# quzefan/LuSh-NeRF

Measured on AMD Instinct MI355X. Metric: training rays/sec (fwd+bwd), N_samples=64+64, higher is better.
Workload: dtype f16 MFMA forward (one fp16 plane per operand, fp32 accumulate; render outputs within 3e-5 of the fp32 reference); backward fp16 MFMA (one plane, per-launch power-of-two loss scale), fp32 accumulate; 1 GPU; poster_lushnerf 1xMI355X N_rand=4096/GPU N_samples=64 N_importance=64 blur kernel (DSK/RBK) on, fwd+bwd+Adam, one RCCL all-reduce of the flat gradient (BASELINE config C2); rays_per_gpu=4096, marched_rays_per_gpu=20480, planes_fwd=fp16x1, parallelism=dp1

## Files before the change

lush_nerf_amd/csrc/lush_abi.hip:

```cpp
#include "lush_common.h"
#include "lush_host.h"
#include <cstring>
#include <vector>
#include "../../include/lush_march.h"

using namespace lush;

namespace {

struct NetInfo { int HW, NL, SKIP, HV, NRB, total_entries, f32_total; };
template <class N> NetInfo info_of() { return {N::HW, N::NL, N::SKIP, N::HV, N::NRB, N::total_entries, N::f32_total}; }
bool net_info(int net, NetInfo& o) {
    if (net == 0) { o = info_of<NetNerf>(); return true; }
    if (net == 1) { o = info_of<NetNoise>(); return true; }
    return false;
}

inline bool code_ok(int c) { return (c >= 1 && c <= 3) || c == PLANES_F16; }
inline int nplanes(int c) { return c == PLANES_F16 ? 1 : c; }
constexpr int PT_PAD = 256;
inline long long pad_pts(long long P) { return (P + PT_PAD - 1) / PT_PAD * PT_PAD; }
inline size_t al256(size_t x) { return (x + 255) & ~(size_t)255; }

struct StashLayout {
    size_t mask, mask_dummy, pe, xd, h[NET_MAX_LAYERS], feat, hv, total;
    long long Ppad;
};
StashLayout stash_layout(const NetInfo& n, int pf, int sp, long long P) {
    StashLayout L{};
    L.Ppad = pad_pts(P);
    size_t off = 0;
    L.mask = off; off += sp ? al256((size_t)(L.Ppad / 32) * (n.NL + 1) * n.NRB * 16 * 8) : 0;
    L.mask_dummy = off; off += sp ? 4096 : 0;
    for (int l = 0; l < n.NL; ++l) { L.h[l] = off; off += al256((size_t)sp * L.Ppad * n.HW * 2); }
    L.feat = off; off += sp >= 3 ? al256((size_t)sp * L.Ppad * n.HW * 2) : 0;
    L.hv = off;   off += al256((size_t)sp * L.Ppad * n.HV * 2);
    L.xd = off;   off += sp ? al256((size_t)L.Ppad * 32) : 0;
    L.pe = off;   off += al256((size_t)pf * L.Ppad * PE_ROW * 2);
    L.total = off;
    return L;
}
struct DStashLayout { size_t scale, fac, dz[NET_MAX_LAYERS], dfeat, dzv, total; };
DStashLayout dstash_layout(const NetInfo& n, int ns, long long P) {
    DStashLayout L{};
    const long long Ppad = pad_pts(P);
    size_t off = 0;
    L.scale = off; off += 256;
    L.fac = off; off += ns <= 2 ? al256((size_t)((n.HV + DZV_EXT) * (n.HW + 1) + DZV_EXT * (n.HV + 1)) * 4) : 0;
    for (int l = 0; l < n.NL; ++l) { L.dz[l] = off; off += al256((size_t)ns * Ppad * n.HW * 2); }
    L.dfeat = off; off += ns >= 3 ? al256((size_t)ns * Ppad * n.HW * 2) : 0;
    L.dzv = off;   off += al256((size_t)ns * Ppad * (n.HV + (ns == 1 ? DZV_EXT : 0)) * 2);
    L.total = off;
    return L;
}

MlpParams to_params(const lush_mlp_params* p) {
    MlpParams q;
    for (int i = 0; i < NET_MAX_LAYERS; ++i) { q.w[i] = p->w[i]; q.b[i] = p->b[i]; }
    q.w_feat = p->w_feat; q.b_feat = p->b_feat; q.w_alpha = p->w_alpha; q.b_alpha = p->b_alpha;
    q.w_views = p->w_views; q.b_views = p->b_views; q.w_rgb = p->w_rgb; q.b_rgb = p->b_rgb;
    return q;
}

template <class N>
void build_pack_table(const lush_mlp_params* p, PackTable& T, int& blocks, int copy_lo, int copy_hi) {
    constexpr int HW = N::HW, HV = N::HV, NL = N::NL, SK = N::SKIP;
    T.n = 0;
    blocks = 0;
    int perm = 0, base = 0;
    auto add = [&](const float* src, int sr, int sk, int rows, int cols, int nrb, int kk, int dst) {
        PackJob& j = T.j[T.n++];
        j.src = src; j.sr = sr; j.sk = sk; j.rows = rows; j.cols = cols; j.nrb = nrb; j.kk = kk; j.perm = perm;
        j.dst_entry = base + dst; j.first_block = blocks;
        blocks += nrb * kk;
    };
    const int XV = PE_X_VALID, DV = PE_D_VALID;
    for (int copy = copy_lo; copy <= copy_hi; ++copy) {
        perm = copy; base = copy ? N::fwd2_base : 0;
        add(p->w[0], XV, 1, HW, XV, N::NRB, N::KKX, N::fwd_L(0, false));
        for (int l = 1; l < NL; ++l) {
            if (l == SK) {
                add(p->w[l], XV + HW, 1, HW, XV, N::NRB, N::KKX, N::fwd_L(l, false));
                add(p->w[l] + XV, XV + HW, 1, HW, HW, N::NRB, N::KKH, N::fwd_L(l, true));
            } else {
                add(p->w[l], HW, 1, HW, HW, N::NRB, N::KKH, N::fwd_L(l, true));
            }
        }
        add(p->w_feat, HW, 1, HW, HW, N::NRB, N::KKH, N::fwd_FEAT);
        add(p->w_alpha, HW, 1, 1, HW, 1, N::KKH, N::fwd_ALPHA);
        add(p->w_views, HW + DV, 1, HV, HW, N::NRBV, N::KKH, N::fwd_VA);
        add(p->w_views + HW, HW + DV, 1, HV, DV, N::NRBV, N::KKD, N::fwd_VB);
        add(p->w_rgb, HV, 1, 3, HV, 1, N::KKV, N::fwd_RGB);
    }
    perm = 0; base = 0;
    for (int copy = copy_lo; copy <= copy_hi; ++copy) {
        perm = copy; base = copy ? N::bwd2_base - N::bwd_VAT : 0;
        add(p->w_views, 1, HW + DV, HW, HV, N::NRB, N::KKV, N::bwd_VAT);
        add(p->w_views + HW, 1, HW + DV, DV, HV, 1, N::KVB, N::bwd_VBT);
        add(p->w_feat, 1, HW, HW, HW, N::NRB, N::KKH, N::bwd_FEATT);
        for (int l = NL - 1; l >= 1; --l) {
            if (l == SK) {
                add(p->w[l], 1, XV + HW, XV, HW, 2, N::KKH, N::bwd_LT(l, false));
                add(p->w[l] + XV, 1, XV + HW, HW, HW, N::NRB, N::KKH, N::bwd_LT(l, true));
            } else {
                add(p->w[l], 1, HW, HW, HW, N::NRB, N::KKH, N::bwd_LT(l, true));
            }
        }
        add(p->w[0], 1, XV, XV, HW, 2, N::KKH, N::bwd_LT(0, false));
    }
    perm = 0; base = 0;
}

template <class N>
void build_pack_table_half(const lush_mlp_params* p, PackTable& T, int& blocks) {
    constexpr int HW = N::HW, HV = N::HV, NL = N::NL, SK = N::SKIP, HR = N::HW / 2, NRBH = N::NRB / 2;
    T.n = 0;
    blocks = 0;
    int dst = N::fwd3_base;
    auto add = [&](const float* src, int sr, int rows, int cols, int nrb, int kk) {
        PackJob& j = T.j[T.n++];
        j.src = src; j.sr = sr; j.sk = 1; j.rows = rows; j.cols = cols; j.nrb = nrb; j.kk = kk; j.perm = 1;
        j.dst_entry = dst; j.first_block = blocks;
        blocks += nrb * kk;
        dst += nrb * kk;
    };
    const int XV = PE_X_VALID, DV = PE_D_VALID;
    for (int half = 0; half < 2; ++half) add(p->w[0] + (long long)half * HR * XV, XV, HR, XV, NRBH, N::KKX);
    for (int l = 1; l < NL; ++l) {
        const int ld = l == SK ? XV + HW : HW;
        for (int half = 0; half < 2; ++half) {
            const float* w = p->w[l] + (long long)half * HR * ld;
            if (l == SK) {
                add(w, ld, HR, XV, NRBH, N::KKX);
                add(w + XV, ld, HR, HW, NRBH, N::KKH);
            } else {
                add(w, ld, HR, HW, NRBH, N::KKH);
            }
        }
    }
    for (int half = 0; half < 2; ++half) add(p->w_feat + (long long)half * HR * HW, HW, HR, HW, NRBH, N::KKH);
    add(p->w_alpha, HW, 1, HW, 1, N::KKH);
    add(p->w_views, HW + DV, HV, HW, N::NRBV, N::KKH);
    add(p->w_views + HW, HW + DV, HV, DV, N::NRBV, N::KKD);
    add(p->w_rgb, HV, 3, HV, 1, N::KKV);
}

template <class N>
void build_pack_table_wide(const lush_mlp_params* p, PackTable& T, int& blocks) {
    constexpr int HW = N::HW, HV = N::HV, NL = N::NL, SK = N::SKIP, QR = 64;
    T.n = 0;
    blocks = 0;
    int dst = N::fwd4_base;
    auto add = [&](const float* src, int sr, int rows, int cols, int nrb, int kk) {
        PackJob& j = T.j[T.n++];
        j.src = src; j.sr = sr; j.sk = 1; j.rows = rows; j.cols = cols; j.nrb = nrb; j.kk = kk; j.perm = 1;
        j.dst_entry = dst; j.first_block = blocks;
        blocks += nrb * kk;
        dst += nrb * kk;
    };
    const int XV = PE_X_VALID, DV = PE_D_VALID;
    for (int q = 0; q < HW / QR; ++q) add(p->w[0] + (long long)q * QR * XV, XV, QR, XV, 2, N::KKX);
    for (int l = 1; l < NL; ++l) {
        const int ld = l == SK ? XV + HW : HW;
        for (int q = 0; q < HW / QR; ++q) {
            const float* w = p->w[l] + (long long)q * QR * ld;
            if (l == SK) {
                add(w, ld, QR, XV, 2, N::KKX);
                add(w + XV, ld, QR, HW, 2, N::KKH);
            } else {
                add(w, ld, QR, HW, 2, N::KKH);
            }
        }
    }
    for (int q = 0; q < HW / QR; ++q) add(p->w_feat + (long long)q * QR * HW, HW, QR, HW, 2, N::KKH);
    add(p->w_alpha, HW, 1, HW, 1, N::KKH);
    for (int q = 0; q < HV / QR; ++q) {
        const float* w = p->w_views + (long long)q * QR * (HW + DV);
        add(w + HW, HW + DV, QR, DV, 2, 4);
        add(w, HW + DV, QR, HW, 2, N::KKH);
    }
    add(p->w_rgb, HV, 3, HV, 1, N::KKV);
}

template <class N>
void build_pack_table_wide_bwd(const lush_mlp_params* p, PackTable& T, int& blocks) {
    constexpr int HW = N::HW, HV = N::HV, NL = N::NL, SK = N::SKIP, QR = 64;
    T.n = 0;
    blocks = 0;
    int dst = N::bwd4_base;
    auto add = [&](const float* src, int sk, int rows, int cols, int nrb, int kk) {
        PackJob& j = T.j[T.n++];
        j.src = src; j.sr = 1; j.sk = sk; j.rows = rows; j.cols = cols; j.nrb = nrb; j.kk = kk; j.perm = 1;
        j.dst_entry = dst; j.first_block = blocks;
        blocks += nrb * kk;
        dst += nrb * kk;
    };
    const int XV = PE_X_VALID, DV = PE_D_VALID;
    for (int q = 0; q < HW / QR; ++q) add(p->w_views + q * QR, HW + DV, QR, HV, 2, N::KKV);
    add(p->w_views + HW, HW + DV, DV, HV, 1, N::KKV);
    for (int q = 0; q < HW / QR; ++q) add(p->w_feat + q * QR, HW, QR, HW, 2, N::KKH);
    for (int l = NL - 1; l >= 1; --l) {
        const int ld = l == SK ? XV + HW : HW;
        for (int q = 0; q < HW / QR; ++q) add(p->w[l] + (l == SK ? XV : 0) + q * QR, ld, QR, HW, 2, N::KKH);
        if (l == SK) add(p->w[l], ld, XV, HW, 2, N::KKH);
    }
    add(p->w[0], XV, XV, HW, 2, N::KKH);
}

template <class N>
void build_pack_table_half_bwd(const lush_mlp_params* p, PackTable& T, int& blocks) {
    constexpr int HW = N::HW, HV = N::HV, NL = N::NL, SK = N::SKIP, HR = N::HW / 2, NRBH = N::NRB / 2;
    T.n = 0;
    blocks = 0;
    int dst = N::bwd3_base;
    auto add = [&](const float* src, int sk, int rows, int cols, int nrb, int kk) {
        PackJob& j = T.j[T.n++];
        j.src = src; j.sr = 1; j.sk = sk; j.rows = rows; j.cols = cols; j.nrb = nrb; j.kk = kk; j.perm = 1;
        j.dst_entry = dst; j.first_block = blocks;
        blocks += nrb * kk;
        dst += nrb * kk;
    };
    const int XV = PE_X_VALID, DV = PE_D_VALID;
    for (int half = 0; half < 2; ++half) add(p->w_views + half * HR, HW + DV, HR, HV, NRBH, N::KKV);
    add(p->w_views + HW, HW + DV, DV, HV, 1, N::KVB);
    for (int half = 0; half < 2; ++half) add(p->w_feat + half * HR, HW, HR, HW, NRBH, N::KKH);
    for (int l = NL - 1; l >= 1; --l) {
        const int ld = l == SK ? XV + HW : HW;
        if (l == SK) add(p->w[l], ld, XV, HW, 2, N::KKH);
        for (int half = 0; half < 2; ++half) add(p->w[l] + (l == SK ? XV : 0) + half * HR, ld, HR, HW, NRBH, N::KKH);
    }
    add(p->w[0], XV, XV, HW, 2, N::KKH);
}

int dw_splits(long long Ppad) {
    int dev = 0, s = 256;
    if (current_device_cus(dev, s) != 0) s = 256;
#ifndef LUSH_DW_MIN_PTS
#define LUSH_DW_MIN_PTS 128
#endif
    const long long max_s = Ppad / LUSH_DW_MIN_PTS > 0 ? Ppad / LUSH_DW_MIN_PTS : 1;
    if (s > max_s) s = (int)max_s;
    return s < 1 ? 1 : s;
}

}

extern "C" {

size_t lush_mlp_packed_bytes(int net, int planes) {
    NetInfo n;
    if (!net_info(net, n) || !code_ok(planes)) return 0;
    return al256((size_t)n.total_entries * nplanes(planes) * 1024 + (size_t)n.f32_total * 4);
}

static int collect_pack_tables(int net, int planes, const lush_mlp_params* prm, int variant, std::vector<PackTable>& out,
                               std::vector<int>& out_blocks) {
    if (!code_ok(planes)) return set_error("lush_mlp_pack: planes must be 1..3 or 17 (fp16)");
    if (net != 0 && net != 1) return set_error("lush_mlp_pack: bad net");
    auto push = [&](const PackTable& T, int blocks) { out.push_back(T); out_blocks.push_back(blocks); };
    PackTable T;
    int blocks = 0;
    const int older = LUSH_VARIANT_FWD_HALF | LUSH_VARIANT_FWD_512 | LUSH_VARIANT_BWD_HALF | LUSH_VARIANT_BWD_512;
    if (net == 0 && planes == PLANES_F16 && variant >= 0 && !(variant & older)) {
        build_pack_table_wide<NetNerf>(prm, T, blocks);
        if (blocks != NetNerf::fwd4_len) return set_error("lush_mlp_pack: quarter-row stream length");
        push(T, blocks);
        build_pack_table_wide_bwd<NetNerf>(prm, T, blocks);
        if (blocks != NetNerf::bwd4_len) return set_error("lush_mlp_pack: transposed quarter-row stream length");
        push(T, blocks);
        return 0;
    }
    const bool fc = mlp_fwd_chain_enabled(planes), bc = mlp_bwd_chain_enabled(planes);
    const int lo = (fc && bc) ? 1 : 0, hi = (fc || bc) ? 1 : 0;
    if (net == 0) build_pack_table<NetNerf>(prm, T, blocks, lo, hi);
    else build_pack_table<NetNoise>(prm, T, blocks, lo, hi);
    push(T, blocks);
    if (net == 0 && nplanes(planes) == 1) {
        build_pack_table_half<NetNerf>(prm, T, blocks);
        push(T, blocks);
        if (planes == PLANES_F16) {
            build_pack_table_half_bwd<NetNerf>(prm, T, blocks);
            push(T, blocks);
            build_pack_table_wide<NetNerf>(prm, T, blocks);
            if (blocks != NetNerf::fwd4_len) return set_error("lush_mlp_pack: quarter-row stream length");
            push(T, blocks);
            build_pack_table_wide_bwd<NetNerf>(prm, T, blocks);
            if (blocks != NetNerf::bwd4_len) return set_error("lush_mlp_pack: transposed quarter-row stream length");
            push(T, blocks);
        }
    }
    return 0;
}

int lush_mlp_pack_for(int net, int planes, const lush_mlp_params* prm, void* packed, int variant, lush_stream_t stream) {
    std::vector<PackTable> tables;
    std::vector<int> blocks;
    int rc = collect_pack_tables(net, planes, prm, variant, tables, blocks);
    for (size_t i = 0; i < tables.size() && !rc; ++i) rc = launch_pack(planes, tables[i], blocks[i], packed, (hipStream_t)stream);
    if (rc) return rc;
    return launch_pack_f32(net, nplanes(planes), to_params(prm), packed, (hipStream_t)stream);
// ... 444 lines not shown
```

lush_nerf_amd/csrc/lush_mlp.h:

```cpp
#pragma once
#include <stdint.h>

namespace lush {

enum { NET_MAX_LAYERS = 8 };
enum { PLANES_F16 = 17 };
enum { LUSH_VARIANT_FWD_HALF = 1, LUSH_VARIANT_FWD_512 = 2, LUSH_VARIANT_BWD_512 = 4, LUSH_VARIANT_HEAD_KERNEL = 8, LUSH_VARIANT_BWD_HALF = 16,
       LUSH_VARIANT_PE_ROWS = 64, LUSH_VARIANT_DW_SPLIT = 128, LUSH_VARIANT_DENSE_BWD = 256, LUSH_VARIANT_DW_WALK = 512,
       LUSH_VARIANT_KERNEL_BITS = 0x3DF };

template <int HW_, int NL_, int SKIP_>
struct NetT {
    static constexpr int HW = HW_, NL = NL_, SKIP = SKIP_;
    static constexpr int HV = HW / 2;
    static constexpr int NRB = HW / 32, NRBV = HV / 32;
    static constexpr int KKH = HW / 16, KKV = HV / 16;
    static constexpr int KKX = 4, KKD = 2;

    static constexpr int fwd_L(int l, bool part_b) {
        int off = 0;
        if (l == 0) return 0;
        off += KKX * NRB;
        for (int i = 1; i < l; ++i) off += (i == SKIP ? (KKX + KKH) : KKH) * NRB;
        if (l == SKIP && part_b) off += KKX * NRB;
        return off;
    }
    static constexpr int fwd_FEAT = fwd_L(NL, false);
    static constexpr int fwd_ALPHA = fwd_FEAT + KKH * NRB;
    static constexpr int fwd_VA = fwd_ALPHA + KKH;
    static constexpr int fwd_VB = fwd_VA + KKH * NRBV;
    static constexpr int fwd_RGB = fwd_VB + KKD * NRBV;
    static constexpr int fwd_END = fwd_RGB + KKV;

    static constexpr int KVB = 2 * NRB;
    static_assert(KVB >= KKV && KVB <= KKH, "VBT padding");
    static constexpr int bwd_VAT = fwd_END;
    static constexpr int bwd_VBT = bwd_VAT + KKV * NRB;
    static constexpr int bwd_FEATT = bwd_VBT + KVB;
    static constexpr int bwd_LT(int l, bool part_b) {
        int off = bwd_FEATT + KKH * NRB;
        for (int i = NL - 1; i > l; --i) off += (i == SKIP ? (KKH * 2 + KKH * NRB) : KKH * NRB);
        if (l == SKIP && part_b) off += KKH * 2;
        return off;
    }
    static constexpr int bwd_END = bwd_LT(0, false) + KKH * 2;
    static constexpr int fwd2_base = bwd_END;
    static constexpr int bwd2_base = fwd2_base + fwd_END;
    static constexpr int fwd3_base = bwd2_base + (bwd_END - bwd_VAT);
    static constexpr int bwd3_base = fwd3_base + fwd_END;
    static constexpr int fwd4_base = bwd3_base + (bwd_END - bwd_VAT);
    static constexpr int fwd4_len = fwd_ALPHA + KKH + (HV / 64) * (8 + 2 * KKH) + KKV;
    static constexpr int bwd4_base = fwd4_base + fwd4_len;
    static constexpr int bwd4_len = (HW / 64) * 2 * KKV + KKV + (HW / 64) * 2 * KKH * NL + (SKIP > 0 ? 2 * KKH : 0) + 2 * KKH;
    static constexpr int total_entries = bwd4_base + bwd4_len;

    static constexpr int n_mask_layers = NL + 1;

    static constexpr int f32_b_trunk = 0;
    static constexpr int f32_b_feat = NL * HW;
    static constexpr int f32_b_alpha = f32_b_feat + HW;
    static constexpr int f32_b_views = f32_b_alpha + 32;
    static constexpr int f32_b_rgb = f32_b_views + HV;
    static constexpr int f32_w_rgb = f32_b_rgb + 32;
    static constexpr int f32_w_alpha = f32_w_rgb + 3 * HV;
    static constexpr int f32_total = f32_w_alpha + HW;
};

typedef NetT<256, 8, 5> NetNerf;
typedef NetT<128, 4, -1> NetNoise;

__host__ __device__ constexpr int chain_row(int rho) {
    const int h = (rho >> 2) & 1, q = (rho & 3) + 4 * (rho >> 3);
    return 16 * (q >> 3) + 8 * h + (q & 7);
}

struct PackJob {
    const float* src;
    int sr, sk;
    int rows, cols;
    int nrb, kk;
    int perm;
    int dst_entry;
    int first_block;
};

struct PackTable {
    PackJob j[64];
    int n;
};

struct PlanJob {
    PackJob j;
    void* dst;
    int code;
    int kind;
    int prm_index;
    int pad;
};
constexpr int PLAN_MAX_NETS = 8;
struct PlanHeader {
    int n_jobs, total_blocks, n_prm, pad;
};

struct MlpParams {
    const float* w[NET_MAX_LAYERS];
    const float* b[NET_MAX_LAYERS];
    const float *w_feat, *b_feat, *w_alpha, *b_alpha, *w_views, *b_views, *w_rgb, *b_rgb;
};

struct MlpGrads {
    float* w[NET_MAX_LAYERS];
    float* b[NET_MAX_LAYERS];
    float *w_feat, *b_feat, *w_alpha, *b_alpha, *w_views, *b_views, *w_rgb, *b_rgb;
};

struct MlpFwdArgs {
    const float* rays;
    const float* z;
    int S, P, n_tiles;
    const uint4* wpk;
    float* raw;
    unsigned long long* mask;
    void* mask_dummy;
    __bf16* pe;
    float* xd;
    int pe_rows;
    __bf16* h0;
    __bf16* feat;
    __bf16* hv;
    long long h_stride;
    long long plane_pe, plane_h, plane_hv;
    int write_stash;
    int stash_planes;
    const int* live_idx;
    const int* live_cnt;
};

struct MlpBwdArgs {
    const float* rays;
    const float* z;
    int S, P, n_tiles;
    const uint4* wpk;
    const float* draw;
    const unsigned long long* mask;
    __bf16* dz0;
    __bf16* dfeat;
    __bf16* dzv;
    long long dz_stride;
    long long plane_h, plane_hv;
    float* dpts;
    const float* scale;
    const int* live_idx;
    const int* live_cnt;
};

struct DwArgs {
    const __bf16* Z; long long z_plane; int ldz; int n_out;
    const __bf16* X; long long x_plane; int ldx; int xcol0; int k_in;
    float* dW; int ldw; int wcol0;
    float* db;
    int x_f16;
    int z_f16;
    const float* scale;
    int Ppad;
    int pts_per_split;
};

// ... 48 lines not shown
```

lush_nerf_amd/csrc/lush_mlp.hip:

```cpp
#include "lush_common.h"
#include "lush_mlp.h"
#include "lush_mlp_dev.h"

namespace lush {

constexpr int DW_THREADS = 256;

template <int NS, int DT>
__device__ __forceinline__ void pack_entry(const PackJob& J, int e, __bf16* __restrict__ dst) {
    const int kk = e / J.nrb, rb = e % J.nrb;
    const int lane = threadIdx.x, r = lane & 31, h = lane >> 5;
    const int row = rb * 32 + (J.perm ? chain_row(r) : r);
    __bf16 out[NS][8];
#pragma unroll
    for (int i = 0; i < 8; ++i) {
        const int k = kk * 16 + 8 * h + i;
        float v = 0.f;
        if (row < J.rows && k < J.cols) v = J.src[(long long)row * J.sr + (long long)k * J.sk];
        __bf16 p[NS];
        split_planes<NS, DT>(v, p);
#pragma unroll
        for (int s = 0; s < NS; ++s) out[s][i] = p[s];
    }
    __bf16* base = dst + ((long long)(J.dst_entry + e) * NS) * 64 * 8;
#pragma unroll
    for (int s = 0; s < NS; ++s) {
        bf16x8 v;
#pragma unroll
        for (int i = 0; i < 8; ++i) v[i] = out[s][i];
        *reinterpret_cast<bf16x8*>(base + ((long long)s * 64 + lane) * 8) = v;
    }
}

template <int NS, int DT>
__global__ __launch_bounds__(64) void pack_kernel(const PackTable T, __bf16* __restrict__ dst) {
    int b = blockIdx.x;
    int j = 0;
    while (j + 1 < T.n && T.j[j + 1].first_block <= b) ++j;
    const PackJob J = T.j[j];
    pack_entry<NS, DT>(J, b - J.first_block, dst);
}

template <class N>
__device__ __forceinline__ float pack_f32_value(const MlpParams& P, int i) {
    float v = 0.f;
    if (i < N::f32_b_feat) v = P.b[i / N::HW][i % N::HW];
    else if (i < N::f32_b_alpha) v = P.b_feat[i - N::f32_b_feat];
    else if (i < N::f32_b_views) v = (i == N::f32_b_alpha) ? P.b_alpha[0] : 0.f;
    else if (i < N::f32_b_rgb) v = P.b_views[i - N::f32_b_views];
    else if (i < N::f32_w_rgb) v = (i - N::f32_b_rgb < 3) ? P.b_rgb[i - N::f32_b_rgb] : 0.f;
    else if (i < N::f32_w_alpha) v = P.w_rgb[i - N::f32_w_rgb];
    else v = P.w_alpha[i - N::f32_w_alpha];
    return v;
}
template <class N>
__global__ void pack_f32_kernel(const MlpParams P, float* __restrict__ dst) {
    const int i = blockIdx.x * blockDim.x + threadIdx.x;
    if (i >= N::f32_total) return;
    dst[i] = pack_f32_value<N>(P, i);
}

__global__ __launch_bounds__(64) void pack_plan_kernel(const PlanHeader* __restrict__ H, float* __restrict__ zero_buf, long long zero_n) {
    if (zero_buf != nullptr) {
        const long long t = (long long)blockIdx.x * 64 + threadIdx.x, nt = (long long)gridDim.x * 64;
        if ((reinterpret_cast<size_t>(zero_buf) & 15) == 0) {
            float4* z4 = reinterpret_cast<float4*>(zero_buf);
            for (long long i = t; i < zero_n / 4; i += nt) z4[i] = make_float4(0.f, 0.f, 0.f, 0.f);
            for (long long i = zero_n / 4 * 4 + t; i < zero_n; i += nt) zero_buf[i] = 0.f;
        } else {
            for (long long i = t; i < zero_n; i += nt) zero_buf[i] = 0.f;
        }
    }
    const MlpParams* prm = reinterpret_cast<const MlpParams*>(H + 1);
    const PlanJob* jobs = reinterpret_cast<const PlanJob*>(prm + PLAN_MAX_NETS);
    const int b = blockIdx.x;
    int lo = 0, hi = H->n_jobs - 1;
    while (lo < hi) {
        const int mid = (lo + hi + 1) >> 1;
        if (jobs[mid].j.first_block <= b) lo = mid; else hi = mid - 1;
    }
    const PlanJob& PJ = jobs[lo];
    const int e = b - PJ.j.first_block;
    if (PJ.kind == 0) {
        const PackJob J = PJ.j;
        __bf16* dst = reinterpret_cast<__bf16*>(PJ.dst);
        if (PJ.code == PLANES_F16) pack_entry<1, DT_F16>(J, e, dst);
        else if (PJ.code == 1) pack_entry<1, DT_BF16>(J, e, dst);
        else if (PJ.code == 2) pack_entry<2, DT_BF16>(J, e, dst);
        else pack_entry<3, DT_BF16>(J, e, dst);
    } else {
        const int i = e * 64 + threadIdx.x;
        float* dst = reinterpret_cast<float*>(PJ.dst);
        if (PJ.kind == 1) { if (i < NetNerf::f32_total) dst[i] = pack_f32_value<NetNerf>(prm[PJ.prm_index], i); }
        else if (i < NetNoise::f32_total) dst[i] = pack_f32_value<NetNoise>(prm[PJ.prm_index], i);
    }
}

template <int NS, int RB, int CB, int KK, int DT = DT_BF16>
__device__ __forceinline__ void seg_gemm(f32x16 (&acc)[RB][CB], const bf16x8* __restrict__ wseg,
                                         int nrb, int rb0, const char* img, int plane_bytes,
                                         int row_bytes, int chunk0, int lane) {
// ... 1617 lines not shown
```

lush_nerf_amd/csrc/lush_mlp_wide_bwd.hip:

```cpp
#include "lush_mlp_wide.h"
#include "lush_host.h"

#include <cstdio>
#include <cstdlib>

namespace lush {

constexpr int WB_WRAP = NetNerf::bwd4_len / 8;
LUSH_CLOCK_DECL(lush_clock_wide_bwd)
#ifdef LUSH_PROF
__device__ unsigned long long lush_prof_wbwd[16];
#define BPROF_T(var) const unsigned long long var = __builtin_amdgcn_s_memtime()
#define BPROF_ADD(slot, t0) cx.prof[slot] += __builtin_amdgcn_s_memtime() - (t0)
#else
#define BPROF_T(var)
#define BPROF_ADD(slot, t0)
#endif
static_assert(NetNerf::bwd4_len % 8 == 0, "the transposed quarter-row stream is whole positions");
constexpr int WB_DPE_LD = 104;
constexpr int WB_TILE_OPS = 6 + 32 + 2 + 16;
constexpr int WB_SB = 2;
enum { WK_NONE = 0, WK_ACT = 1, WK_ID = 2 };

struct WbRt {
    unsigned mrd;
    const float* initw;
    float dalpha[2];
    const char* msrc[2];
    unsigned mdst;
    char* tile;
    const char* lut;
    char* srows;
    unsigned srow_off;
};

struct WbConvTmp {
    unsigned w[4];
    u32x4 Y[2];
    unsigned o[4];
};

enum { WI_L = 0, WI_P = 1, WI_ID = 2, WI_IA = 3, WI_IB = 4 };
struct WbItem { int kind, b, t, i; };

template <int NRQ, int NPOS, int CK, int CKB0, bool INIT, bool ZERO, int D, int PQ, bool STASH, int LD, bool MDMA, int XP = 0>
struct WbPass {
    static constexpr int KBPP = 8 / NRQ;
    static constexpr int NG = NPOS * 16;
    static constexpr int DG = D < NG ? D : NG;
    struct Seq { WbItem it[128]; int n; };
    static constexpr Seq make_seq() {
        Seq q{};
        q.n = 0;
        auto put = [&](int kind, int b, int t, int i) { q.it[q.n].kind = kind; q.it[q.n].b = b; q.it[q.n].t = t; q.it[q.n].i = i; ++q.n; };
        auto init = [&](int b) {
            if (INIT) {
                for (int j = 0; j < 4; ++j) put(WI_IA, b, 0, j);
                for (int j = 0; j < 4; ++j) put(WI_IB, b, 0, j);
            }
        };
        if (CK == WK_ACT) {
            put(WI_L, 0, 0, 0);
            for (int bt = 0; bt < 8; ++bt) {
                if (bt + 1 < 8) put(WI_L, (bt + 1) / 2, (bt + 1) % 2, 0);
                for (int i = 0; i < 4; ++i) put(WI_P, bt / 2, bt % 2, i);
                if (bt % 2 == 1) init(bt / 2);
            }
        } else if (CK == WK_ID) {
            for (int bt = 0; bt < 8; ++bt) {
                for (int i = 0; i < 4; ++i) put(WI_ID, bt / 2, bt % 2, i);
                if (bt % 2 == 1) init(bt / 2);
            }
        } else {
            for (int b = 0; b < 4; ++b) init(b);
        }
        return q;
    }
    static constexpr Seq SQ = make_seq();
    static constexpr int NIT = SQ.n;
    static constexpr int START = CK == WK_ACT ? 2 : 0;
    static_assert(!STASH || NPOS == 4, "the stash pipeline is laid out over the 16 positions of a layer");

    struct Regs {
        bf16x8 a1[4];
        WbConvTmp ct;
        unsigned dma_dst, dma_off;
    };

    static constexpr int ST_JOBS = 8;
    static constexpr bool st_write(int g) { return STASH && g % 16 >= 12 && (4 * PQ + g / 16) < ST_JOBS; }
    static constexpr bool st_read(int g) { return STASH && g % 16 >= 12 && (4 * PQ + g / 16) >= 1 && (4 * PQ + g / 16) <= ST_JOBS; }
// ... 330 lines not shown
        const unsigned voff_row = (unsigned)(((lane >> 3) * LD_ + (lane & 7) * 8) * 2);
#pragma unroll
        for (int i = 0; i < 4; ++i) {
            const int row = 8 * i + (lane >> 3);
            const u32x4 v = *reinterpret_cast<const u32x4*>(rt.tile + row * 128 + (((lane & 7) ^ (row & 7)) << 4));
            asm volatile("global_store_dwordx4 %0, %1, %2 nt\n\ts_nop 1" ::"v"(voff_row), "v"(v), "s"(rows + ((c * 32 + 8 * i) * LD_ + j * 64) * 2) : "memory");
        }
    };

    f32x4 drn[2];
    auto prefetch = [&](int t) __attribute__((always_inline)) {
        const long long wp = (long long)t * WD_MT + row0;
        const char* mb0 = wd_uniform(reinterpret_cast<const char*>(A.mask) + (wp / 32) * CB_BYTES - w * 1024);
        wd_dma_pair(mb0 + NL * 1024, mb0 + CB_BYTES + NL * 1024, cx.voff, mbuf_lds + (NL % 2) * 2048u, mbuf_lds + (NL % 2) * 2048u + 1024u);
        wd_dma_pair(mb0 + (NL - 1) * 1024, mb0 + CB_BYTES + (NL - 1) * 1024, cx.voff, mbuf_lds + ((NL - 1) % 2) * 2048u, mbuf_lds + ((NL - 1) % 2) * 2048u + 1024u);
#pragma unroll
        for (int c = 0; c < 2; ++c) {
            long long gpt = wp + c * 32 + n;
            if (gpt >= P) gpt = P - 1;
            asm volatile("global_load_dwordx4 %0, %1, %2" : "=v"(drn[c]) : "v"((unsigned)(gpt * 16)), "s"(A.draw) : "memory");
        }
    };
    if ((int)blockIdx.x < n_tiles) prefetch(blockIdx.x);
    asm volatile("s_waitcnt vmcnt(0)" : "+v"(drn[0]), "+v"(drn[1])::"memory");
#ifdef LUSH_PROF
    for (int i = 0; i < 16; ++i) cx.prof[i] = 0;
    const unsigned long long t_kernel = __builtin_amdgcn_s_memtime();
#endif

    for (int tile = blockIdx.x; tile < n_tiles; tile += gridDim.x) {
        const long long pt0 = (long long)tile * WD_MT;
        const long long wpt = pt0 + row0;
        BPROF_T(t_tile);
        {
            unsigned long long gb = (unsigned long long)cx.gbase;
            asm volatile("" : "+s"(gb));
            cx.gbase = (const char*)gb;
        }
        const char* mbase[2];
#pragma unroll
        for (int c = 0; c < 2; ++c) mbase[c] = wd_uniform(reinterpret_cast<const char*>(A.mask) + (wpt / 32 + c) * CB_BYTES - w * 1024);
        asm volatile("s_waitcnt vmcnt(32)" : "+v"(drn[0]), "+v"(drn[1])::"memory");
        float4 dr[2];
#pragma unroll
        for (int c = 0; c < 2; ++c) {
            const bool in = wpt + c * 32 + n < P;
            dr[c].x = in ? drn[c][0] * gscale : 0.f; dr[c].y = in ? drn[c][1] * gscale : 0.f;
            dr[c].z = in ? drn[c][2] * gscale : 0.f; dr[c].w = in ? drn[c][3] * gscale : 0.f;
            rt.dalpha[c] = dr[c].w;
        }
        BPROF_ADD(1, t_tile);
        BPROF_T(t_bar);
        lds_barrier();
        BPROF_ADD(2, t_bar);
        BPROF_T(t_pro);

        f32x16 accA[2][2], accB[2][2];
        u32x4 B0[2][16], B1[2][16];
        WdCarry a0;
#pragma unroll
        for (int i = 0; i < 4; ++i) a0.a0[i] = *reinterpret_cast<const bf16x8*>(cx.ring + cx.slot_off + i * 1024 + cx.voff);

#ifndef LUSH_ABL_NOPRO
        {
            auto rank3 = [&](f32x16 (&acc)[2][2], int r0) __attribute__((always_inline)) {
#pragma unroll
                for (int rbl = 0; rbl < 2; ++rbl)
#pragma unroll
                    for (int j = 0; j < 4; ++j) {
                        const int f = r0 + rbl * 32 + 8 * h + (j == 0 ? 0 : j == 1 ? 4 : j == 2 ? 16 : 20);
                        const f32x4 wr = *reinterpret_cast<const f32x4*>(w_rgb + f);
                        const f32x4 wg = *reinterpret_cast<const f32x4*>(w_rgb + HV + f);
                        const f32x4 wb = *reinterpret_cast<const f32x4*>(w_rgb + 2 * HV + f);
#pragma unroll
                        for (int c = 0; c < 2; ++c)
#pragma unroll
                            for (int e = 0; e < 4; ++e) acc[c][rbl][4 * j + e] = wr[e] * dr[c].x + wg[e] * dr[c].y + wb[e] * dr[c].z;
                    }
            };
            rank3(accA, 0);
            rank3(accB, 64);
            const unsigned m8 = mrd0 + (NL % 2) * 2048;
            rt.mrd = m8;
            WbPass<2, 1, WK_ACT, 0, false, true, 16, 0, false, HW, false>::convert_now(accA, B1, rt, cx.voff);
            rt.mrd = m8 + 2 * 128;
            WbPass<2, 1, WK_ACT, 4, false, true, 16, 0, false, HW, false>::convert_now(accB, B1, rt, cx.voff);
        }
        if (h == 0) {
#pragma unroll
            for (int c = 0; c < 2; ++c) {
                const float4 d = dr[c];
                unsigned a[1], b[1], e[1], f[1];
                split_pair<1, DT_F16>(d.x, d.y, a);
                split_pair<1, DT_F16>(d.z, d.w, b);
                const float hx = elem_to_f32<DT_F16>(__builtin_bit_cast(__bf16, (unsigned short)(a[0] & 0xFFFFu)));
                const float hy = elem_to_f32<DT_F16>(__builtin_bit_cast(__bf16, (unsigned short)(a[0] >> 16)));
                const float hz = elem_to_f32<DT_F16>(__builtin_bit_cast(__bf16, (unsigned short)(b[0] & 0xFFFFu)));
                const float hw = elem_to_f32<DT_F16>(__builtin_bit_cast(__bf16, (unsigned short)(b[0] >> 16)));
                split_pair<1, DT_F16>(d.x - hx, d.y - hy, e);
                split_pair<1, DT_F16>(d.z - hz, d.w - hw, f);
                u32x4 v;
                v[0] = a[0]; v[1] = b[0]; v[2] = e[0]; v[3] = f[0];
                *reinterpret_cast<u32x4*>(A.dzv + (wpt + c * 32 + n) * LDV + HV) = v;
            }
        }
        {
            const char* rows = wd_uniform(reinterpret_cast<const char*>(A.dzv + wpt * LDV));
#pragma unroll
            for (int c = 0; c < 2; ++c)
#pragma unroll
                for (int j = 0; j < N::KKV / 4; ++j) stash_now(B1, c, j, rows, LDV);
        }
#endif
        BPROF_ADD(3, t_pro);
        BPROF_T(t_body);
        if (tile == (int)blockIdx.x) wd_wait_vm<0>();
        static_assert(WD_S - 1 == 5, "the first S - 1 positions of a tile: VA0, VA1 and the first of VA2");
        WbPass<2, 2, WK_NONE, 0, false, true, 32, 0, false, HW, false, 2>::run(cx, accA, accB, B1, B0, a0, rt);
        WbPass<2, 2, WK_ID, 0, false, true, 28, 0, false, HW, false, 2>::run(cx, accB, accA, B1, B0, a0, rt);
        WbPass<2, 2, WK_ID, 4, false, true, 28, 0, false, HW, false, 1>::run(cx, accA, accB, B1, B0, a0, rt);
        WbPass<2, 2, WK_ID, 8, false, true, 28, 0, false, HW, false>::run(cx, accB, accA, B1, B0, a0, rt);
        WbPass<1, 1, WK_ID, 12, false, true, 16, 0, false, HW, false>::run(cx, accA, accB, B1, B0, a0, rt);
#pragma unroll
        for (int c = 0; c < 2; ++c) dpe_put(accA[c][0], c, 2);
#pragma unroll
        for (int c = 0; c < 2; ++c)
#pragma unroll
            for (int rbl = 0; rbl < 2; ++rbl)
#pragma unroll
                for (int j = 0; j < 4; ++j) {
                    const f32x4 v = *reinterpret_cast<const f32x4*>(w_alpha + 8 * h + rbl * 32 + (j == 0 ? 0 : j == 1 ? 4 : j == 2 ? 16 : 20));
#pragma unroll
                    for (int e = 0; e < 4; ++e) accA[c][rbl][4 * j + e] = v[e] * rt.dalpha[c];
                }
        {
            const unsigned m7 = mrd0 + ((NL - 1) % 2) * 2048;
            rt.initw = w_alpha + 8 * h + 64;
            WbPass<2, 4, WK_NONE, 0, true, false, 60, 0, false, HW, false>::run(cx, accA, accB, B0, B1, a0, rt);
            rt.initw = w_alpha + 8 * h + 128; rt.mrd = m7;
            rt.msrc[0] = mbase[0] + (NL - 2) * 1024; rt.msrc[1] = mbase[1] + (NL - 2) * 1024; rt.mdst = mbuf_lds + ((NL - 2) % 2) * 2048u;
            WbPass<2, 4, WK_ACT, 0, true, false, 60, 1, false, HW, true>::run(cx, accB, accA, B0, B1, a0, rt);
            rt.initw = w_alpha + 8 * h + 192; rt.mrd = m7 + 2 * 128;
            WbPass<2, 4, WK_ACT, 4, true, false, 60, 2, false, HW, false>::run(cx, accA, accB, B0, B1, a0, rt);
            rt.mrd = m7 + 4 * 128;
            WbPass<2, 4, WK_ACT, 8, false, false, 60, 3, false, HW, false>::run(cx, accB, accA, B0, B1, a0, rt);
        }
        auto layer = [&](int l, u32x4 (&xin)[2][16], u32x4 (&xout)[2][16]) __attribute__((always_inline)) {
            const unsigned ml = mrd0 + (unsigned)(l % 2) * 2048u;
            const unsigned mo = mrd0 + (unsigned)((l - 1) % 2) * 2048u;
            rt.srows = const_cast<char*>(wd_uniform(reinterpret_cast<const char*>(A.dz0 + (long long)l * A.dz_stride + wpt * HW)));
            rt.mrd = ml + 6 * 128;
            WbPass<2, 4, WK_ACT, 12, false, true, 48, 0, true, HW, false>::run(cx, accA, accB, xin, xin, a0, rt);
            rt.mrd = mo;
            {
                const int mn = l >= 2 ? l - 2 : 0;
                rt.msrc[0] = mbase[0] + mn * 1024; rt.msrc[1] = mbase[1] + mn * 1024; rt.mdst = mbuf_lds + (unsigned)(l % 2) * 2048u;
            }
            WbPass<2, 4, WK_ACT, 0, false, true, 60, 1, true, HW, true>::run(cx, accB, accA, xin, xout, a0, rt);
            rt.mrd = mo + 2 * 128;
            WbPass<2, 4, WK_ACT, 4, false, true, 60, 2, true, HW, false>::run(cx, accA, accB, xin, xout, a0, rt);
            rt.mrd = mo + 4 * 128;
            WbPass<2, 4, WK_ACT, 8, false, true, 60, 3, true, HW, false>::run(cx, accB, accA, xin, xout, a0, rt);
        };
#pragma unroll 1
        for (int l2 = 0; l2 < NL / 2; ++l2) {
            const int l = NL - 1 - 2 * l2;
            layer(l, B1, B0);
            if (l == N::SKIP) {
                WbPass<2, 4, WK_NONE, 0, false, true, 64, 0, false, HW, false>::run(cx, accA, accB, B1, B1, a0, rt);
#pragma unroll
                for (int c = 0; c < 2; ++c) { dpe_put(accA[c][0], c, 0); dpe_put(accA[c][1], c, 1); }
            }
            if (l > 1) layer(l - 1, B0, B1);
        }
        float px[3] = {0.f, 0.f, 0.f}, pd[3] = {0.f, 0.f, 0.f};
        if (wpt + lane < P) point_of(A.rays, A.z, A.S, A.live_idx ? (long long)A.live_idx[wpt + lane] : wpt + lane, px, pd);
        rt.mrd = mrd0 + 6 * 128;
        WbPass<2, 4, WK_ACT, 12, false, true, 48, 0, false, HW, false>::run(cx, accA, accB, B0, B0, a0, rt);
        BPROF_ADD(4, t_body);
        BPROF_T(t_epi);
#ifndef LUSH_ABL_NOEPI
#pragma unroll
        for (int c = 0; c < 2; ++c) {
            dpe_add(accA[c][0], c, 0); dpe_add(accA[c][1], c, 1);
            dpe_put(accA[c][0], c, 0); dpe_put(accA[c][1], c, 1);
        }
        float rvh[3], rvl[3], rdh[3], rdl[3];
#pragma unroll
        for (int i = 0; i < 3; ++i) {
            rev_split(px[i], &rvh[i], &rvl[i]);
            rev_split(pd[i], &rdh[i], &rdl[i]);
            asm volatile("" : "+v"(rvh[i]), "+v"(rvl[i]), "+v"(rdh[i]), "+v"(rdl[i]));
        }
        prefetch(tile + (int)gridDim.x < n_tiles ? tile + (int)gridDim.x : tile);
        {
            const char* rows = wd_uniform(reinterpret_cast<const char*>(A.dz0 + wpt * HW));
#pragma unroll
            for (int c = 0; c < 2; ++c)
#pragma unroll
                for (int j = 0; j < 4; ++j) stash_now(B0, c, j, rows, HW);
        }
        BPROF_ADD(9, t_epi);
        BPROF_T(t_enc);
        {
            const __bf16* g = dpe + (row0 + lane) * WB_DPE_LD;
            float gv[PE_X + PE_D];
#pragma unroll
            for (int cc = 0; cc < (PE_X + PE_D) / 8; ++cc) {
                const bf16x8 v = *reinterpret_cast<const bf16x8*>(g + 8 * cc);
#pragma unroll
                for (int e = 0; e < 8; ++e) gv[8 * cc + e] = elem_to_f32<DT_F16>(v[e]);
            }
            float gx[3], gd[3];
#pragma unroll
            for (int i = 0; i < 3; ++i) {
                const float hx = rvh[i], lx = rvl[i], hd = rdh[i], ld = rdl[i];
                float sx = gv[i], sd = gv[PE_X + i];
#pragma unroll
                for (int k = 0; k < L_X; ++k) {
                    float sn, cs;
                    sincos_rev(hx, lx, k, &sn, &cs);
                    sx += (float)(1 << k) * (cs * gv[3 + 6 * k + i] - sn * gv[3 + 6 * k + 3 + i]);
                }
#pragma unroll
                for (int k = 0; k < L_D; ++k) {
                    float sn, cs;
                    sincos_rev(hd, ld, k, &sn, &cs);
                    sd += (float)(1 << k) * (cs * gv[PE_X + 3 + 6 * k + i] - sn * gv[PE_X + 3 + 6 * k + 3 + i]);
                }
// ... 54 lines not shown
```

Baseline: 349,600 rays/s.

## Fold views-by-feature weight product into backward pack, removing feature-layer backward GEMM

The weight packer gains a fold mode that precomputes the product of the view-layer weights and the feature-layer weights on device. The wide backward kernel then applies this folded matrix directly to the view-layer gradient, skipping the separate backward pass through the feature layer. The pass schedule is restructured to match: the alpha-gradient init moves before the tile body, the pass list is rebalanced, and bwd4_len shrinks by one layer's worth of entries. This removes one hidden-width backward GEMM per tile in exchange for a small extra matmul in weight packing. It also changes how rounding error accumulates in fp16, since the product is formed in fp32 before quantization.

After: 352,000 rays/s (median of 6 runs). About the same (+0.7%).

```diff
diff --git a/lush_nerf_amd/csrc/lush_abi.hip b/lush_nerf_amd/csrc/lush_abi.hip
--- a/lush_nerf_amd/csrc/lush_abi.hip
+++ b/lush_nerf_amd/csrc/lush_abi.hip
@@ -71,6 +71,7 @@
     auto add = [&](const float* src, int sr, int sk, int rows, int cols, int nrb, int kk, int dst) {
         PackJob& j = T.j[T.n++];
         j.src = src; j.sr = sr; j.sk = sk; j.rows = rows; j.cols = cols; j.nrb = nrb; j.kk = kk; j.perm = perm;
+        j.fold = 0; j.src2 = nullptr;
         j.dst_entry = base + dst; j.first_block = blocks;
         blocks += nrb * kk;
     };
@@ -120,6 +121,7 @@
     auto add = [&](const float* src, int sr, int rows, int cols, int nrb, int kk) {
         PackJob& j = T.j[T.n++];
         j.src = src; j.sr = sr; j.sk = 1; j.rows = rows; j.cols = cols; j.nrb = nrb; j.kk = kk; j.perm = 1;
+        j.fold = 0; j.src2 = nullptr;
         j.dst_entry = dst; j.first_block = blocks;
         blocks += nrb * kk;
         dst += nrb * kk;
@@ -154,6 +156,7 @@
     auto add = [&](const float* src, int sr, int rows, int cols, int nrb, int kk) {
         PackJob& j = T.j[T.n++];
         j.src = src; j.sr = sr; j.sk = 1; j.rows = rows; j.cols = cols; j.nrb = nrb; j.kk = kk; j.perm = 1;
+        j.fold = 0; j.src2 = nullptr;
         j.dst_entry = dst; j.first_block = blocks;
         blocks += nrb * kk;
         dst += nrb * kk;
@@ -191,14 +194,19 @@
     auto add = [&](const float* src, int sk, int rows, int cols, int nrb, int kk) {
         PackJob& j = T.j[T.n++];
         j.src = src; j.sr = 1; j.sk = sk; j.rows = rows; j.cols = cols; j.nrb = nrb; j.kk = kk; j.perm = 1;
+        j.fold = 0; j.src2 = nullptr;
         j.dst_entry = dst; j.first_block = blocks;
         blocks += nrb * kk;
         dst += nrb * kk;
     };
     const int XV = PE_X_VALID, DV = PE_D_VALID;
-    for (int q = 0; q < HW / QR; ++q) add(p->w_views + q * QR, HW + DV, QR, HV, 2, N::KKV);
+    static_assert(HW <= PACK_FOLD_MAX, "folded sum length");
+    for (int q = 0; q < HW / QR; ++q) {
+        add(p->w_views, HW + DV, QR, HV, 2, N::KKV);
+        PackJob& j = T.j[T.n - 1];
+        j.fold = HW; j.src2 = p->w_feat + q * QR; j.sr = HW;
+    }
     add(p->w_views + HW, HW + DV, DV, HV, 1, N::KKV);
-    for (int q = 0; q < HW / QR; ++q) add(p->w_feat + q * QR, HW, QR, HW, 2, N::KKH);
     for (int l = NL - 1; l >= 1; --l) {
         const int ld = l == SK ? XV + HW : HW;
         for (int q = 0; q < HW / QR; ++q) add(p->w[l] + (l == SK ? XV : 0) + q * QR, ld, QR, HW, 2, N::KKH);
@@ -216,6 +224,7 @@
     auto add = [&](const float* src, int sk, int rows, int cols, int nrb, int kk) {
         PackJob& j = T.j[T.n++];
         j.src = src; j.sr = 1; j.sk = sk; j.rows = rows; j.cols = cols; j.nrb = nrb; j.kk = kk; j.perm = 1;
+        j.fold = 0; j.src2 = nullptr;
         j.dst_entry = dst; j.first_block = blocks;
         blocks += nrb * kk;
         dst += nrb * kk;
diff --git a/lush_nerf_amd/csrc/lush_mlp.h b/lush_nerf_amd/csrc/lush_mlp.h
--- a/lush_nerf_amd/csrc/lush_mlp.h
+++ b/lush_nerf_amd/csrc/lush_mlp.h
@@ -51,7 +51,7 @@
     static constexpr int fwd4_base = bwd3_base + (bwd_END - bwd_VAT);
     static constexpr int fwd4_len = fwd_ALPHA + KKH + (HV / 64) * (8 + 2 * KKH) + KKV;
     static constexpr int bwd4_base = fwd4_base + fwd4_len;
-    static constexpr int bwd4_len = (HW / 64) * 2 * KKV + KKV + (HW / 64) * 2 * KKH * NL + (SKIP > 0 ? 2 * KKH : 0) + 2 * KKH;
+    static constexpr int bwd4_len = (HW / 64) * 2 * KKV + KKV + (HW / 64) * 2 * KKH * (NL - 1) + (SKIP > 0 ? 2 * KKH : 0) + 2 * KKH;
     static constexpr int total_entries = bwd4_base + bwd4_len;
 
     static constexpr int n_mask_layers = NL + 1;
@@ -82,7 +82,10 @@
     int perm;
     int dst_entry;
     int first_block;
-};
+    int fold;
+    const float* src2;
+};
+constexpr int PACK_FOLD_MAX = 256;
 
 struct PackTable {
     PackJob j[64];
diff --git a/lush_nerf_amd/csrc/lush_mlp.hip b/lush_nerf_amd/csrc/lush_mlp.hip
--- a/lush_nerf_amd/csrc/lush_mlp.hip
+++ b/lush_nerf_amd/csrc/lush_mlp.hip
@@ -12,11 +12,30 @@
     const int lane = threadIdx.x, r = lane & 31, h = lane >> 5;
     const int row = rb * 32 + (J.perm ? chain_row(r) : r);
     __bf16 out[NS][8];
+    float f[8] = {0.f, 0.f, 0.f, 0.f, 0.f, 0.f, 0.f, 0.f};
+    if (J.fold > 0) {
+        __shared__ __attribute__((aligned(16))) float sa[16][PACK_FOLD_MAX + 4];
+        for (int t = lane; t < 16 * J.fold; t += 64) {
+            const int kr = t / J.fold, j = t - kr * J.fold, k = kk * 16 + kr;
+            sa[kr][j] = k < J.cols ? J.src[(long long)k * J.sk + j] : 0.f;
+        }
+        __syncthreads();
+        if (row < J.rows) {
+            const float* b = J.src2 + row;
+#pragma unroll 4
+            for (int j = 0; j < J.fold; ++j) {
+                const float bj = b[(long long)j * J.sr];
+#pragma unroll
+                for (int i = 0; i < 8; ++i) f[i] = fmaf(sa[8 * h + i][j], bj, f[i]);
+            }
+        }
+    }
 #pragma unroll
     for (int i = 0; i < 8; ++i) {
         const int k = kk * 16 + 8 * h + i;
         float v = 0.f;
-        if (row < J.rows && k < J.cols) v = J.src[(long long)row * J.sr + (long long)k * J.sk];
+        if (J.fold > 0) v = f[i];
+        else if (row < J.rows && k < J.cols) v = J.src[(long long)row * J.sr + (long long)k * J.sk];
         __bf16 p[NS];
         split_planes<NS, DT>(v, p);
 #pragma unroll
diff --git a/lush_nerf_amd/csrc/lush_mlp_wide_bwd.hip b/lush_nerf_amd/csrc/lush_mlp_wide_bwd.hip
--- a/lush_nerf_amd/csrc/lush_mlp_wide_bwd.hip
+++ b/lush_nerf_amd/csrc/lush_mlp_wide_bwd.hip
@@ -7,6 +7,7 @@
 namespace lush {
 
 constexpr int WB_WRAP = NetNerf::bwd4_len / 8;
+static_assert(WB_WRAP == 129, "the tile's pass list below consumes 129 positions");
 LUSH_CLOCK_DECL(lush_clock_wide_bwd)
 #ifdef LUSH_PROF
 __device__ unsigned long long lush_prof_wbwd[16];
@@ -503,9 +504,9 @@
             rank3(accB, 64);
             const unsigned m8 = mrd0 + (NL % 2) * 2048;
             rt.mrd = m8;
-            WbPass<2, 1, WK_ACT, 0, false, true, 16, 0, false, HW, false>::convert_now(accA, B1, rt, cx.voff);
+            WbPass<2, 1, WK_ACT, 0, false, true, 16, 0, false, HW, false>::convert_now(accA, B0, rt, cx.voff);
             rt.mrd = m8 + 2 * 128;
-            WbPass<2, 1, WK_ACT, 4, false, true, 16, 0, false, HW, false>::convert_now(accB, B1, rt, cx.voff);
+            WbPass<2, 1, WK_ACT, 4, false, true, 16, 0, false, HW, false>::convert_now(accB, B0, rt, cx.voff);
         }
         if (h == 0) {
 #pragma unroll
@@ -530,42 +531,41 @@
 #pragma unroll
             for (int c = 0; c < 2; ++c)
 #pragma unroll
-                for (int j = 0; j < N::KKV / 4; ++j) stash_now(B1, c, j, rows, LDV);
-        }
-#endif
+                for (int j = 0; j < N::KKV / 4; ++j) stash_now(B0, c, j, rows, LDV);
+        }
+#endif
+#pragma unroll
+        for (int c = 0; c < 2; ++c)
+#pragma unroll
+            for (int rbl = 0; rbl < 2; ++rbl)
+#pragma unroll
+                for (int j = 0; j < 4; ++j) {
+                    const f32x4 v = *reinterpret_cast<const f32x4*>(w_alpha + 8 * h + rbl * 32 + (j == 0 ? 0 : j == 1 ? 4 : j == 2 ? 16 : 20));
+#pragma unroll
+                    for (int e = 0; e < 4; ++e) accA[c][rbl][4 * j + e] = v[e];
+                    asm volatile("v_mul_f32 %0, %0, %4\n\tv_mul_f32 %1, %1, %4\n\tv_mul_f32 %2, %2, %4\n\tv_mul_f32 %3, %3, %4"
+                                 : "+v"(accA[c][rbl][4 * j]), "+v"(accA[c][rbl][4 * j + 1]), "+v"(accA[c][rbl][4 * j + 2]), "+v"(accA[c][rbl][4 * j + 3])
+                                 : "v"(rt.dalpha[c]));
+                }
         BPROF_ADD(3, t_pro);
         BPROF_T(t_body);
         if (tile == (int)blockIdx.x) wd_wait_vm<0>();
         static_assert(WD_S - 1 == 5, "the first S - 1 positions of a tile: VA0, VA1 and the first of VA2");
-        WbPass<2, 2, WK_NONE, 0, false, true, 32, 0, false, HW, false, 2>::run(cx, accA, accB, B1, B0, a0, rt);
-        WbPass<2, 2, WK_ID, 0, false, true, 28, 0, false, HW, false, 2>::run(cx, accB, accA, B1, B0, a0, rt);
-        WbPass<2, 2, WK_ID, 4, false, true, 28, 0, false, HW, false, 1>::run(cx, accA, accB, B1, B0, a0, rt);
-        WbPass<2, 2, WK_ID, 8, false, true, 28, 0, false, HW, false>::run(cx, accB, accA, B1, B0, a0, rt);
-        WbPass<1, 1, WK_ID, 12, false, true, 16, 0, false, HW, false>::run(cx, accA, accB, B1, B0, a0, rt);
-#pragma unroll
-        for (int c = 0; c < 2; ++c) dpe_put(accA[c][0], c, 2);
-#pragma unroll
-        for (int c = 0; c < 2; ++c)
-#pragma unroll
-            for (int rbl = 0; rbl < 2; ++rbl)
-#pragma unroll
-                for (int j = 0; j < 4; ++j) {
-                    const f32x4 v = *reinterpret_cast<const f32x4*>(w_alpha + 8 * h + rbl * 32 + (j == 0 ? 0 : j == 1 ? 4 : j == 2 ? 16 : 20));
-#pragma unroll
-                    for (int e = 0; e < 4; ++e) accA[c][rbl][4 * j + e] = v[e] * rt.dalpha[c];
-                }
         {
             const unsigned m7 = mrd0 + ((NL - 1) % 2) * 2048;
             rt.initw = w_alpha + 8 * h + 64;
-            WbPass<2, 4, WK_NONE, 0, true, false, 60, 0, false, HW, false>::run(cx, accA, accB, B0, B1, a0, rt);
+            WbPass<2, 2, WK_NONE, 0, true, false, 30, 0, false, HW, false, 2>::run(cx, accA, accB, B0, B1, a0, rt);
             rt.initw = w_alpha + 8 * h + 128; rt.mrd = m7;
             rt.msrc[0] = mbase[0] + (NL - 2) * 1024; rt.msrc[1] = mbase[1] + (NL - 2) * 1024; rt.mdst = mbuf_lds + ((NL - 2) % 2) * 2048u;
-            WbPass<2, 4, WK_ACT, 0, true, false, 60, 1, false, HW, true>::run(cx, accB, accA, B0, B1, a0, rt);
+            WbPass<2, 2, WK_ACT, 0, true, false, 30, 0, false, HW, true, 2>::run(cx, accB, accA, B0, B1, a0, rt);
             rt.initw = w_alpha + 8 * h + 192; rt.mrd = m7 + 2 * 128;
-            WbPass<2, 4, WK_ACT, 4, true, false, 60, 2, false, HW, false>::run(cx, accA, accB, B0, B1, a0, rt);
+            WbPass<2, 2, WK_ACT, 4, true, false, 30, 0, false, HW, false, 1>::run(cx, accA, accB, B0, B1, a0, rt);
             rt.mrd = m7 + 4 * 128;
-            WbPass<2, 4, WK_ACT, 8, false, false, 60, 3, false, HW, false>::run(cx, accB, accA, B0, B1, a0, rt);
-        }
+            WbPass<2, 2, WK_ACT, 8, false, false, 30, 0, false, HW, false>::run(cx, accB, accA, B0, B1, a0, rt);
+            WbPass<1, 1, WK_NONE, 0, false, true, 16, 0, false, HW, false>::run(cx, accA, accB, B0, B1, a0, rt);
+        }
+#pragma unroll
+        for (int c = 0; c < 2; ++c) dpe_put(accA[c][0], c, 2);
         auto layer = [&](int l, u32x4 (&xin)[2][16], u32x4 (&xout)[2][16]) __attribute__((always_inline)) {
             const unsigned ml = mrd0 + (unsigned)(l % 2) * 2048u;
             const unsigned mo = mrd0 + (unsigned)((l - 1) % 2) * 2048u;
```
